# pkorus/neural-imaging

Hardware: AMD Instinct MI355X
Metric: patches/s (fwd+bwd) ISP->JPEG->FAN @256^2 (higher is better)
Workload: dtype bf16; 1 GPU; c4 = train_manipulation UNet->[native,sharpen:1,resample:50,gaussian:0.83,jpeg:80]->dJPEG(QF80,soft)->FAN, ds none, trainable nip+fan, lambda_nip 0.1; raw_patch=128, batch_per_gpu=64, global_batch=64, parallelism=dp1, world_size=1, hip_graph=False

## Files before the change

### include/nimg.h

```cpp
#ifndef NIMG_H
#define NIMG_H

#include <stddef.h>
#include <stdint.h>

#ifdef __cplusplus
extern "C" {
#endif

#define NIMG_OK 0
#define NIMG_ERR_ARG (-1)
#define NIMG_ERR_LAUNCH (-2)
#define NIMG_ERR_WORKSPACE (-3)

#define NIMG_BF16_IN 1
#define NIMG_BF16_OUT 2
#define NIMG_BF16_MASK 4
#define NIMG_BF16_DZ 8
#define NIMG_D2S_OUT 16
#define NIMG_MASK_CONV 128
#define NIMG_COPY_LRELU 64
#define NIMG_S2D_OUT 32
#define NIMG_UNPOOL_OUT 512
#define NIMG_D2S_CONVT 1024
// ... 252 lines not shown
                            float* out1, int o1, float* out2, int o2, const float* act_mask, int n, int h, int wd,
                            int ks, int stride, int pad_t, int pad_l, int pad_mode, int hout, int wout, int act,
                            float alpha, int flags, void* stream);
int nimg_conv2d_wgrad_bf16_ex(const float* in1, int c1, const float* in2, int c2, const float* dz, int cout, float* dw,
                              float* db, int n, int h, int wd, int ks, int stride, int pad_t, int pad_l, int pad_mode,
                              int hout, int wout, int accumulate, void* workspace, size_t workspace_bytes, int flags,
                              void* stream);
int nimg_conv2d_pool_fwd_bf16_ex(const float* in, int cin, const float* w, const void* wb, const float* bias,
                                 float* pool_out, unsigned char* pool_idx, int cout, int n, int h, int wd, int ks,
                                 int act, float alpha, int flags, void* stream);
int nimg_conv2d_fwd_pool_also_bf16(const float* in, int cin, const void* wb, const float* bias, float* out, float* pool_out,
                                   unsigned char* pool_idx, int cout, int n, int h, int wd, int act, float alpha, void* stream);
#define NIMG_ROWS_F32_OUT 1
int nimg_conv3_rows_bf16(const void* in1, int c1, const void* in2, int c2, const void* wb, const float* bias, const void* mask,
                         void* out, void* out2, void* pool_out, int n, int h, int wd, int cout, int act, float alpha, int flags,
                         void* stream);
int nimg_conv3_rows_d2s_bf16(const void* in, int c1, const void* wb, const float* bias, float* y, int n, int h, int wd, void* stream);
int nimg_conv3_rows_c4_bf16(const float* in, const float* w, const float* bias, void* out, int n, int h, int wd, int act, float alpha,
                            void* stream);

int nimg_conv2d_dgrad_unpool_out_bf16(const float* dz, int c1, const void* wb, const float* act, const float* skip, float* out,
                                      int cout, int n, int h, int wd, int apply_mask, float alpha, void* stream);
int nimg_conv2d_wgrad_pooled_bf16_ex(const float* in, int cin, const float* g, const unsigned char* idx, int cout,
                                     float* dw, float* db, int n, int h, int wd, int ks, int accumulate, void* workspace,
                                     size_t workspace_bytes, int flags, void* stream);
int nimg_conv2d_dgrad_fewin_pooled_bf16_ex(const float* g, const unsigned char* idx, const float* w, float* out, int ci,
                                           int cz, int n, int h, int wd, int ks, int flags, void* stream);
int nimg_maxpool2_unpool_ex(const float* dp, const unsigned char* idx, const float* pooled, float* dz, int n, int ho,
                            int wo, int c, int apply_lrelu_mask, float alpha, int flags, void* stream);
int nimg_convt2x2_fwd_bf16(const float* x, const void* wb, const float* bias, float* y, int n, int h, int wd, int cin,
                           int cout, void* stream);
int nimg_convt2x2_fwd_bf16_ex(const float* x, const void* wb, const float* bias, float* y, int n, int h, int wd, int cin,
                              int cout, int flags, void* stream);
int nimg_conv_weights_bf16_batch(const void* table, int n_entries, void* stream);
int nimg_conv2d_fwd_bf16(const float* in1, int c1, const float* in2, int c2, const void* wb, const float* bias,
                         float* out1, int o1, float* out2, int o2, const float* act_mask, int n, int h, int wd,
                         int ks, int stride, int pad_t, int pad_l, int pad_mode, int hout, int wout, int act,
                         float alpha, void* stream);
size_t nimg_conv2d_wgrad_bf16_workspace_bytes(int cin, int cout, int ks_h, int ks_w, int n, int hout, int wout);
int nimg_conv2d_wgrad_bf16(const float* in1, int c1, const float* in2, int c2, const float* dz, int cout, float* dw,
                           float* db, int n, int h, int wd, int ks, int stride, int pad_t, int pad_l, int pad_mode,
                           int hout, int wout, int accumulate, void* workspace, size_t workspace_bytes, void* stream);

int nimg_conv2d_fwd_smallc_bf16(const float* in, int cin, const float* w, const float* bias, float* out, int cout,
                                int n, int h, int wd, int ks, int pad_mode, int act, float alpha, void* stream);
int nimg_conv2d_fwd_smallc_bf16_ex(const float* in, int cin, const float* w, const float* bias, float* out, int cout,
                                   int n, int h, int wd, int ks, int pad_mode, int act, float alpha, int flags, void* stream);
int nimg_conv2d_dgrad_fewin_bf16(const float* dz, const float* w, float* out, int ci, int cz, int n, int h, int wd,
                                 int ks, void* stream);

int nimg_awgn_fwd(const float* x, const float* noise, float* y, uint8_t* mask, long count, float strength,
                  void* stream);
int nimg_awgn_bwd(const float* x, const float* noise, const float* dy, const uint8_t* mask, float* dx, long count,
                  float strength, void* stream);
int nimg_gamma_fwd(const float* x, float* y, long count, float gamma, void* stream);
int nimg_gamma_bwd(const float* x, const float* dy, float* dx, long count, float gamma, void* stream);
int nimg_median_fwd(const float* x, float* y, uint8_t* sel, int n, int h, int w, int kernel, void* stream);
int nimg_median_bwd(const float* dy, const uint8_t* sel, float* dx, int n, int h, int w, int kernel, void* stream);

#define NIMG_L3IC_E_READ 1
#define NIMG_L3IC_E_LANES 2
#define NIMG_L3IC_E_RANGE 4
#define NIMG_L3IC_E_SYMBOL 8
#define NIMG_L3IC_E_FREQ 16
#define NIMG_L3IC_E_VARINT 32
#define NIMG_L3IC_E_ODD 64
// ... 120 lines not shown
```

### neural-imaging_amd/csrc/common.h

```cpp
#pragma once
#include <hip/hip_runtime.h>
#include <stdint.h>
#include "../../include/nimg.h"

#define NIMG_CHECK_LAUNCH()                                   \
    do {                                                      \
        hipError_t e__ = hipGetLastError();                   \
        if (e__ != hipSuccess) return NIMG_ERR_LAUNCH;        \
    } while (0)

namespace nimg {

constexpr int WAVE = 64;

typedef __bf16 nimg_bf16x4 __attribute__((ext_vector_type(4)));

__device__ __forceinline__ float lrelu(float v, float alpha) { return v > 0.0f ? v : alpha * v; }

typedef unsigned short nimg_u16x2 __attribute__((ext_vector_type(2)));
__device__ __forceinline__ unsigned bf16x2_positive(unsigned packed) {
    const nimg_u16x2 one = {1, 1}, inf = {0x7F80, 0x7F80};
    const nimg_u16x2 u = __builtin_bit_cast(nimg_u16x2, packed) - one;
    return __builtin_bit_cast(unsigned, __builtin_elementwise_min(__builtin_elementwise_sub_sat(inf, u), one));
}
__device__ __forceinline__ unsigned sign_bits_interleave(unsigned x) {
    x = (x | (x << 4)) & 0x0F0F0F0Fu;
    x = (x | (x << 2)) & 0x33333333u;
    x = (x | (x << 1)) & 0x55555555u;
    return (x | (x >> 15)) & 0xFFFFu;
}

__device__ __forceinline__ float wave_sum(float v) {
#pragma unroll
    for (int o = 32; o > 0; o >>= 1) v += __shfl_xor(v, o, 64);
    return v;
}

__device__ __forceinline__ double wave_sum_d(double v) {
#pragma unroll
    for (int o = 32; o > 0; o >>= 1) v += __shfl_xor(v, o, 64);
    return v;
}

__device__ __forceinline__ bool map_coord(int& g, int size, int pad_mode) {
    const bool inside = (unsigned)g < (unsigned)size;
    const int sym = g < 0 ? -1 - g : 2 * size - 1 - g;
    const int ref = g < 0 ? -g : 2 * size - 2 - g;
    const int m = pad_mode == 1 ? sym : ref;
    const bool mapped = pad_mode != 0 && (unsigned)m < (unsigned)size;
    g = inside ? g : (mapped ? m : g);
    return inside || mapped;
}

__device__ __forceinline__ int xcd_order(int bid) {
#ifdef NIMG_NO_XCD_ORDER
    return bid;
#else
    const int g = (int)gridDim.x, x = bid & 7, r = g & 7;
    return x * (g >> 3) + (x < r ? x : r) + (bid >> 3);
#endif
}

typedef float nimg_f32x16 __attribute__((ext_vector_type(16)));

constexpr int EPI_PAD = 4;
template <int NI, bool BLOCK_SYNC = true, typename Emit>
__device__ __forceinline__ void epilogue_via_lds(const nimg_f32x16 (&acc)[NI], float* lds, int lane, Emit emit) {
    constexpr int RS = NI * 32 + EPI_PAD;
    const int half = lane >> 5, n = lane & 31;
    if (BLOCK_SYNC) __syncthreads();
    else __builtin_amdgcn_wave_barrier();
#pragma unroll
    for (int ni = 0; ni < NI; ++ni)
#pragma unroll
        for (int j = 0; j < 16; ++j) lds[((j & 3) + 8 * (j >> 2) + 4 * half) * RS + ni * 32 + n] = acc[ni][j];
    if (BLOCK_SYNC) __syncthreads();
    else __builtin_amdgcn_wave_barrier();
#pragma unroll
    for (int it = 0; it < (32 * NI * 8) / 64; ++it) {
        const int idx = it * 64 + lane, row = idx / (NI * 8), c4 = idx % (NI * 8);
        const float4 v = *reinterpret_cast<const float4*>(lds + row * RS + c4 * 4);
        emit(row, c4 * 4, v);
    }
}

template <int NI, bool BLOCK_SYNC = true, typename Bias, typename Emit>
__device__ __forceinline__ void pool_via_lds(const nimg_f32x16 (&acc)[NI], float* lds, int lane, float alpha, Bias bias4,
                                             Emit emit) {
    constexpr int RS = NI * 32 + EPI_PAD;
    const int half = lane >> 5, n = lane & 31;
    if (BLOCK_SYNC) __syncthreads();
    else __builtin_amdgcn_wave_barrier();
#pragma unroll
    for (int ni = 0; ni < NI; ++ni)
// ... 375 lines not shown
```

### neural-imaging_amd/csrc/conv_bf16_wgrad.hip

```cpp
#include "conv_bf16_wgrad.h"

namespace {

typedef short s16x4 __attribute__((ext_vector_type(4)));
typedef short s16x8 __attribute__((ext_vector_type(8)));

__device__ __forceinline__ bf16x8 tr_read8(const unsigned char* p0, const unsigned char* p1) {
    const s16x4 lo = __builtin_amdgcn_ds_read_tr16_b64_v4i16((s16x4 __attribute__((address_space(3)))*)p0);
    const s16x4 hi = __builtin_amdgcn_ds_read_tr16_b64_v4i16((s16x4 __attribute__((address_space(3)))*)p1);
    s16x8 r;
    r[0] = lo[0]; r[1] = lo[1]; r[2] = lo[2]; r[3] = lo[3]; r[4] = hi[0]; r[5] = hi[1]; r[6] = hi[2]; r[7] = hi[3];
    return *reinterpret_cast<bf16x8*>(&r);
}

constexpr int B_ZS = 192;

template <int KS, int STRIDE, int NW, bool INB, bool DZB, int TH, bool UNP = false, int NCO = 2, bool PAIR = false>
__global__ __launch_bounds__(NW * 64, 2) void conv_wgrad_bf16_kernel(const WgradParamsB p) {
    nimg::reduce_entry_inline(p.pre);
    constexpr int TCO = 32 * NCO, ZS = NCO == 2 ? B_ZS : 64, ZI = 4 * NCO;
    static_assert(NCO == 1 || NCO == 2, "one or two output fragments");
    static_assert(!UNP || NCO == 2, "un-pooling dz: 64-wide tile");
    static_assert(!UNP || (DZB && STRIDE == 1), "un-pooling dz: bf16-stored pooled gradient, stride 1");
    constexpr int TAPS = KS * KS, NT = (TAPS + NW - 1) / NW, NTHR = NW * 64;
    static_assert(!PAIR || (KS == 3 && STRIDE == 1 && TH == 8 && INB && DZB && !UNP), "image pairs: the 3x3 layers over 8 x 8 bf16 images");
    constexpr int THH = (TH - 1) * STRIDE + KS, TWH = PAIR ? 20 : (B_TW - 1) * STRIDE + KS;
    constexpr int NPIXH = THH * TWH, NPIX = TH * B_TW;
    static_assert(STRIDE == 1 || STRIDE == 2, "stride");
    extern __shared__ __attribute__((aligned(16))) unsigned char smem_raw[];
    unsigned char* sI = smem_raw;
    unsigned char* sZ = smem_raw + NPIXH * 64;
    const int tid = threadIdx.x, lane = tid & 63;
    const int wave = __builtin_amdgcn_readfirstlane(tid >> 6);
    const int Cin = p.C1 + p.C2;
    const int cib = (Cin + B_CI - 1) / B_CI, cob = (p.Cout + TCO - 1) / TCO;
    int bid = xcd_order(blockIdx.x);
    const int ci0 = (bid % cib) * B_CI;
    bid /= cib;
    const int co0 = (bid % cob) * TCO;
    const int split = bid / cob;
    const int half = lane >> 5, g = lane & 15, sub = (lane >> 4) & 1;

    f32x16 acc[NT][NCO];
#pragma unroll
    for (int t = 0; t < NT; ++t)
#pragma unroll
        for (int ni = 0; ni < NCO; ++ni)
#pragma unroll
            for (int j = 0; j < 16; ++j) acc[t][ni][j] = 0.0f;
    const int tiles = p.tiles_y * p.tiles_x;
    const int work_total = PAIR ? (p.N + 1) / 2 : p.N * tiles;
    const int w_begin = split * p.work_per_split;
    const int w_end = min(work_total, w_begin + p.work_per_split);
    const bool do_bias = p.db_partial && ci0 == 0;
    float bacc[8] = {0.f, 0.f, 0.f, 0.f, 0.f, 0.f, 0.f, 0.f};
    const int a_lane = ((half * (PAIR ? 10 : 8) + (g >> 2)) * STRIDE) * 64 + (sub * 16 + (g & 3) * 4) * 2;
    const int z_lane = (half * 8 + (g >> 2)) * ZS + (sub * 16 + (g & 3) * 4) * 2;
    constexpr int IP = (NPIXH * 4 + NTHR - 1) / NTHR, ZP = (NPIX * ZI) / NTHR;
    static_assert((NPIX * ZI) % NTHR == 0 && NTHR % ZI == 0, "dz tile must divide over the threads");
    float4 preI[IP][2], preZ[ZP][2];
    uint2 preZK[UNP ? ZP : 1];
    auto fetch = [&](int wk_) {
        const int n_ = (int)(wk_ / tiles), tile_ = (int)(wk_ % tiles);
        const int ty_ = (tile_ / p.tiles_x) * TH, tx_ = (tile_ % p.tiles_x) * B_TW;
        const int iy_ = ty_ * STRIDE - p.pad_t, ix_ = tx_ * STRIDE - p.pad_l;
#pragma unroll
        for (int q = 0; q < IP; ++q) {
            const int item = tid + q * NTHR;
            const int pix = item >> 2, c = ci0 + (item & 3) * 8;
            int gy = iy_ + pix / TWH, gx = ix_ + pix % TWH;
            int ni_ = n_;
            if constexpr (PAIR) {
                const int hx = pix % TWH;
                ni_ = 2 * wk_ + (hx >= 10 ? 1 : 0);
                gx = (hx >= 10 ? hx - 10 : hx) - 1;
                gy = pix / TWH - 1;
            }
            preI[q][0] = preI[q][1] = make_float4(0.f, 0.f, 0.f, 0.f);
            if (item < NPIXH * 4 && c < Cin && (!PAIR || ni_ < p.N) && map_coord(gy, p.H, p.pad_mode) && map_coord(gx, p.W, p.pad_mode)) {
                const long pixoff = ((long)ni_ * p.H + gy) * p.W + gx;
                if constexpr (INB) {
                    const __bf16* src = c < p.C1 ? reinterpret_cast<const __bf16*>(p.in1) + pixoff * p.C1 + c
                                                 : reinterpret_cast<const __bf16*>(p.in2) + pixoff * p.C2 + (c - p.C1);
                    preI[q][0] = *reinterpret_cast<const float4*>(src);
                } else {
                    const float* src = c < p.C1 ? p.in1 + pixoff * p.C1 + c : p.in2 + pixoff * p.C2 + (c - p.C1);
                    preI[q][0] = *reinterpret_cast<const float4*>(src);
// ... 111 lines not shown
        float* red = reinterpret_cast<float*>(smem_raw);
        if (wave > 0) {
#pragma unroll
            for (int ni = 0; ni < 2; ++ni)
#pragma unroll
                for (int j = 0; j < 16; ++j) red[(((wave - 1) * 2 + ni) * 16 + j) * 64 + lane] = acc[0][ni][j];
        }
        __syncthreads();
        if (wave == 0) {
#pragma unroll
            for (int w = 1; w < NW; ++w)
#pragma unroll
                for (int ni = 0; ni < 2; ++ni)
#pragma unroll
                    for (int j = 0; j < 16; ++j) acc[0][ni][j] += red[(((w - 1) * 2 + ni) * 16 + j) * 64 + lane];
        }
    }
    float* slab = p.partial + (long)split * TAPS * Cin * p.Cout;
#pragma unroll
    for (int t = 0; t < NT; ++t) {
        const int tap = KS == 1 ? 0 : wave + NW * t;
        if (tap >= TAPS || (KS == 1 && wave > 0)) continue;
#pragma unroll
        for (int ni = 0; ni < NCO; ++ni) {
            const int co = co0 + ni * 32 + (lane & 31);
            if (co >= p.Cout) continue;
#pragma unroll
            for (int j = 0; j < 16; ++j) {
                const int ci = ci0 + (j & 3) + 8 * (j >> 2) + 4 * half;
                if (ci < Cin) slab[((long)tap * Cin + ci) * p.Cout + co] = acc[t][ni][j];
            }
        }
    }
    if (p.tickets == nullptr) return;
    TicketJob job;
    job.cnt = p.tickets + (long)(xcd_order(blockIdx.x) % (cib * cob)) * ticket_words_per_tile_dev(p.splits, p.group);
    job.slab[0] = p.partial; job.stride[0] = (long)TAPS * Cin * p.Cout; job.dst[0] = p.dw;
    job.slab[1] = p.db_partial; job.stride[1] = p.Cout; job.dst[1] = p.db;
    job.splits = p.splits; job.group = p.group; job.accumulate = p.accumulate;
    const int rows = min(B_CI, Cin - ci0), c4n = min(TCO, p.Cout - co0) >> 2, Cout = p.Cout;
    const int witems = TAPS * rows * c4n;
    const int items = witems + ((p.db_partial && ci0 == 0) ? c4n : 0);
    ticket_finish<NTHR>(job, split, items, [=](int it) {
        TicketItem m;
        if (it >= witems) { m.which = 1; m.off = co0 + (it - witems) * 4; return m; }
        const int c4 = it % c4n, row = it / c4n;
        m.which = 0;
        m.off = ((long)(row / rows) * Cin + ci0 + row % rows) * Cout + co0 + c4 * 4;
        return m;
    }, reinterpret_cast<unsigned*>(smem_raw));
}

int splits_for(int cin, int cout, int n, int hout, int wout, int th = B_TH, int target_blocks = 512) {
    const long blocks_io = (long)cdiv(cin, B_CI) * cdiv(cout, B_CO);
    const long work = (long)n * cdiv(hout, th) * cdiv(wout, B_TW);
    long splits = (target_blocks + blocks_io - 1) / blocks_io;
    if (splits > work) splits = work;
    if (splits < 1) splits = 1;
    const long wps = (work + splits - 1) / splits;
    return (int)((work + wps - 1) / wps);
}

}

extern "C" {

size_t nimg_conv2d_wgrad_bf16_workspace_bytes(int cin, int cout, int ks_h, int ks_w, int n, int hout, int wout) {
    if (cin <= 0 || cout <= 0 || n <= 0) return 0;
    const size_t slab = (size_t)ks_h * ks_w * cin * cout * sizeof(float);
    const size_t generic = (slab + cout * sizeof(float)) * splits_for(cin, cout, n, hout, wout);
    const size_t packed = cin <= 4 ? (4 * slab + cout * sizeof(float)) * nimg_internal_wgrad_packed_splits(cout, n, hout, wout) : 0;
    const size_t tiny = (cin <= 4 && cout <= 4) ? nimg_internal_wgrad_tiny_bytes(ks_h, cin, cout) : 0;
    const size_t m = generic > packed ? generic : packed;
    return m > tiny ? m : tiny;
}

struct ReducePlan {
    nimg::ReduceEntry* defer = nullptr;
    const nimg::ReduceEntry* pre = nullptr;
};
static inline void finish_reduce2(const ReducePlan& plan, const float* p1, float* d1, long n1, int splits1, const float* p2,
                                  float* d2, long n2, int splits2, int accumulate, hipStream_t s) {
    if (plan.defer) nimg::fill_reduce_entry(plan.defer, p1, d1, n1, splits1, p2, d2, n2, splits2, accumulate);
    else launch_reduce2(p1, d1, n1, splits1, p2, d2, n2, splits2, accumulate, s);
}
struct OwedReduction {
    const nimg::ReduceEntry* e;
    hipStream_t s;
    void ran_in_kernel() { e = nullptr; }
    void now() {
        if (e && e->n1 > 0 && e->p1 && e->d1)
            launch_reduce2(e->p1, e->d1, e->n1, e->splits1, e->p2, e->d2, e->n2, e->splits2, e->accumulate, s);
        e = nullptr;
// ... 141 lines not shown
    } while (0)
    if (stride == 1 && ks == 1) NIMG_WGB(1, 1);
    else if (stride == 1 && ks == 3) NIMG_WGB(3, 1);
    else if (stride == 1 && ks == 5) NIMG_WGB(5, 1);
    else if (stride == 2 && ks == 2) NIMG_WGB(2, 2);
    else if (stride == 2 && ks == 5) NIMG_WGB(5, 2);
    else return NIMG_ERR_ARG;
#undef NIMG_WGB
#undef NIMG_WGB1
    NIMG_CHECK_LAUNCH();
    owed.ran_in_kernel();
    if (p.tickets) return NIMG_OK;
    finish_reduce2(plan, (const float*)workspace, dw, count, p.splits, db ? (const float*)p.db_partial : nullptr, db, (long)cout,
                   p.splits, accumulate, s);
    NIMG_CHECK_LAUNCH();
    return NIMG_OK;
}

int nimg_conv2d_wgrad_bf16(const float* in1, int c1, const float* in2, int c2, const float* dz, int cout, float* dw,
                           float* db, int n, int h, int wd, int ks, int stride, int pad_t, int pad_l, int pad_mode,
                           int hout, int wout, int accumulate, void* workspace, size_t workspace_bytes, void* stream) {
    return wgrad_bf16_impl(in1, c1, in2, c2, dz, nullptr, cout, dw, db, n, h, wd, ks, stride, pad_t, pad_l, pad_mode, hout,
                           wout, accumulate, workspace, workspace_bytes, 0, stream, ReducePlan{});
}

int nimg_conv2d_wgrad_bf16_ex(const float* in1, int c1, const float* in2, int c2, const float* dz, int cout, float* dw,
                              float* db, int n, int h, int wd, int ks, int stride, int pad_t, int pad_l, int pad_mode,
                              int hout, int wout, int accumulate, void* workspace, size_t workspace_bytes, int flags,
                              void* stream) {
    return wgrad_bf16_impl(in1, c1, in2, c2, dz, nullptr, cout, dw, db, n, h, wd, ks, stride, pad_t, pad_l, pad_mode, hout,
                           wout, accumulate, workspace, workspace_bytes, flags, stream, ReducePlan{});
}

int nimg_conv2d_wgrad_bf16_unpool(const void* in, int cin, const void* g, const unsigned char* idx, int cout, float* dw, float* db,
                                  int n, int h, int wd, int ks, int accumulate, void* workspace, size_t workspace_bytes,
                                  void* stream) {
    if (!idx || ks != 5 || (h & 1) || (wd & 1)) return NIMG_ERR_ARG;
    return wgrad_bf16_impl((const float*)in, cin, nullptr, 0, (const float*)g, idx, cout, dw, db, n, h, wd, ks, 1, 2, 2, 0, h, wd,
                           accumulate, workspace, workspace_bytes, NIMG_BF16_IN | NIMG_BF16_DZ, stream, ReducePlan{});
}

int nimg_conv2d_wgrad_bf16_deferred(const void* in1, int c1, const void* in2, int c2, const void* dz, const unsigned char* idx,
                                    int cout, float* dw, float* db, int n, int h, int wd, int ks, int stride, int pad_t, int pad_l,
                                    int pad_mode, int hout, int wout, void* workspace, size_t workspace_bytes, int flags,
                                    void* entry, void* stream) {
    if (!entry) return NIMG_ERR_ARG;
    nimg::ReduceEntry* e = reinterpret_cast<nimg::ReduceEntry*>(entry);
    nimg::fill_reduce_entry(e, nullptr, nullptr, 0, 0, nullptr, nullptr, 0, 0, 0);
    e->blocks1 = 0;
    return wgrad_bf16_impl((const float*)in1, c1, (const float*)in2, c2, (const float*)dz, idx, cout, dw, db, n, h, wd, ks, stride,
                           pad_t, pad_l, pad_mode, hout, wout, 0, workspace, workspace_bytes, flags, stream, ReducePlan{e, nullptr});
}

int nimg_conv2d_wgrad_bf16_chained(const void* in1, int c1, const void* in2, int c2, const void* dz, const unsigned char* idx,
                                   int cout, float* dw, float* db, int n, int h, int wd, int ks, int stride, int pad_t, int pad_l,
                                   int pad_mode, int hout, int wout, void* workspace, size_t workspace_bytes, int flags,
                                   const void* pre_entry, void* entry, void* stream) {
    if (!entry) return NIMG_ERR_ARG;
    nimg::ReduceEntry pre_copy;
    if (pre_entry) pre_copy = *reinterpret_cast<const nimg::ReduceEntry*>(pre_entry);
    nimg::ReduceEntry* e = reinterpret_cast<nimg::ReduceEntry*>(entry);
    *e = nimg::empty_reduce_entry();
    return wgrad_bf16_impl((const float*)in1, c1, (const float*)in2, c2, (const float*)dz, idx, cout, dw, db, n, h, wd, ks, stride,
                           pad_t, pad_l, pad_mode, hout, wout, 0, workspace, workspace_bytes, flags, stream,
                           ReducePlan{e, pre_entry ? &pre_copy : nullptr});
}
// ... 42 lines not shown
```

### neural-imaging_amd/csrc/conv_wgrad.hip

```cpp
#include "common.h"

namespace {

using namespace nimg;
typedef float f32x16 __attribute__((ext_vector_type(16)));

struct WgradParams {
    const float* in1;
    const float* in2;
    const float* dz;
    float* partial;
    float* db_partial;
    int C1, C2, Cout;
    int N, H, W, Hout, Wout, pad_t, pad_l;
    int tiles_y, tiles_x, splits, work_per_split, pad_mode;
    int tap0;
};

constexpr int WG_TH = 8, WG_TW = 16;
constexpr int CI_T = 32, CO_T = 64;

template <int KS, int STRIDE, bool VEC, int NW, int TCH = KS * KS>
__global__ __launch_bounds__(NW * 64, 2) void conv_wgrad_kernel(const WgradParams p) {
    constexpr int TAPS = KS * KS, NTHR = NW * 64;
    constexpr int NT = (TCH + NW - 1) / NW;
    constexpr bool PASSES = TCH < TAPS;
    const int tap_first = PASSES ? p.tap0 : 0, tap_end = PASSES ? min(TAPS, p.tap0 + TCH) : TAPS;
    constexpr int THH = (WG_TH - 1) * STRIDE + KS, TWH = (WG_TW - 1) * STRIDE + KS;
    constexpr int NPIXH = THH * TWH, NPIX = WG_TH * WG_TW;
    extern __shared__ __attribute__((aligned(16))) float smem[];
    float* sI = smem;
    float* sZ = smem + NPIXH * CI_T;

// ... 205 lines not shown
            if (co >= p.Cout) continue;
#pragma unroll
            for (int j = 0; j < 16; ++j) {
                const int i = (j & 3) + 8 * (j >> 2) + 4 * (lane >> 5);
                const int tl = i / CINP, ci = i % CINP, tap = f * TPF + tl;
                if (tl < TPF && tap < TAPS) slab[((long)tap * CINP + ci) * p.Cout + co] = acc[f][ni][j];
            }
        }
}

__global__ __launch_bounds__(256) void bias_grad_partial_kernel(const float* __restrict__ dz,
                                                                float* __restrict__ partial, long npix, int cout,
                                                                long pix_per_block) {
    extern __shared__ float red[];
    const int tid = threadIdx.x;
    const int cpad = cout >= 256 ? 256 : (cout > 128 ? 256 : (cout > 64 ? 128 : (cout > 32 ? 64 : 32)));
    const int phases = 256 / cpad;
    const int c = tid % cpad, ph = tid / cpad;
    const long p0 = (long)blockIdx.x * pix_per_block, p1 = min(npix, p0 + pix_per_block);
    for (int cb = 0; cb < cout; cb += cpad) {
        float s = 0.f;
        if (cb + c < cout)
            for (long px = p0 + ph; px < p1; px += phases) s += dz[px * cout + cb + c];
        red[tid] = s;
        __syncthreads();
        if (ph == 0 && cb + c < cout) {
            for (int k = 1; k < phases; ++k) s += red[k * cpad + c];
            partial[(long)blockIdx.x * cout + cb + c] = s;
        }
        __syncthreads();
    }
}

typedef __bf16 bg_bf16x4 __attribute__((ext_vector_type(4)));
template <bool BF>
struct BiasSrc {
    const void* base;
    __device__ __forceinline__ float4 operator[](long i) const {
        if constexpr (BF) {
            const bg_bf16x4 v = reinterpret_cast<const bg_bf16x4*>(base)[i];
            return make_float4((float)v[0], (float)v[1], (float)v[2], (float)v[3]);
        } else {
            return reinterpret_cast<const float4*>(base)[i];
        }
    }
};
template <bool BF>
__global__ __launch_bounds__(256) void bias_grad_partial4_kernel(const float* __restrict__ dz,
                                                                 float* __restrict__ partial, long npix, int cout,
                                                                 long pix_per_block) {
    __shared__ float4 red4[256];
    const int tid = threadIdx.x, cq = cout >> 2, phases = 256 / cq;
    const int c = tid % cq, ph = tid / cq;
    const long p0 = (long)blockIdx.x * pix_per_block, p1 = min(npix, p0 + pix_per_block);
    const BiasSrc<BF> srcb{dz};
    float4 a0 = make_float4(0.f, 0.f, 0.f, 0.f), a1 = a0, a2 = a0, a3 = a0;
    long px = p0 + ph;
    for (; px + 3L * phases < p1; px += 4L * phases) {
        const float4 v0 = srcb[px * cq + c], v1 = srcb[(px + phases) * cq + c], v2 = srcb[(px + 2L * phases) * cq + c],
                     v3 = srcb[(px + 3L * phases) * cq + c];
        a0.x += v0.x; a0.y += v0.y; a0.z += v0.z; a0.w += v0.w;
        a1.x += v1.x; a1.y += v1.y; a1.z += v1.z; a1.w += v1.w;
        a2.x += v2.x; a2.y += v2.y; a2.z += v2.z; a2.w += v2.w;
        a3.x += v3.x; a3.y += v3.y; a3.z += v3.z; a3.w += v3.w;
    }
    for (; px < p1; px += phases) {
        const float4 v = srcb[px * cq + c];
        a0.x += v.x; a0.y += v.y; a0.z += v.z; a0.w += v.w;
    }
    red4[tid] = make_float4((a0.x + a1.x) + (a2.x + a3.x), (a0.y + a1.y) + (a2.y + a3.y),
                            (a0.z + a1.z) + (a2.z + a3.z), (a0.w + a1.w) + (a2.w + a3.w));
    __syncthreads();
    if (ph == 0) {
        float4 s = red4[c];
        for (int k = 1; k < phases; ++k) {
            const float4 v = red4[k * cq + c];
            s.x += v.x; s.y += v.y; s.z += v.z; s.w += v.w;
        }
        reinterpret_cast<float4*>(partial + (long)blockIdx.x * cout)[c] = s;
    }
}

}

extern "C" {

static int wgrad_splits(int cin, int cout, int n, int hout, int wout) {
    const long blocks_io = (long)nimg::cdiv(cin, CI_T) * nimg::cdiv(cout, CO_T);
    const long work = (long)n * nimg::cdiv(hout, WG_TH) * nimg::cdiv(wout, WG_TW);
    long splits = (512 + blocks_io - 1) / blocks_io;
    if (splits > work) splits = work;
    if (splits < 1) splits = 1;
    const long wps = (work + splits - 1) / splits;
    return (int)((work + wps - 1) / wps);
}

static int packed_splits(int cout, int n, int hout, int wout) {
    const long blocks_io = nimg::cdiv(cout, cout <= 32 ? 32 : 64);
    const long work = (long)n * nimg::cdiv(hout, WG_TH) * nimg::cdiv(wout, WG_TW);
    long splits = (512 + blocks_io - 1) / blocks_io;
    if (splits > work) splits = work;
    if (splits < 1) splits = 1;
    const long wps = (work + splits - 1) / splits;
    return (int)((work + wps - 1) / wps);
}

size_t nimg_conv2d_wgrad_workspace_bytes(int cin, int cout, int ks_h, int ks_w, int n, int hout, int wout) {
    if (cin <= 0 || cout <= 0 || n <= 0) return 0;
    const size_t slab = (size_t)ks_h * ks_w * cin * cout * sizeof(float);
    const size_t generic = (slab + cout * sizeof(float)) * wgrad_splits(cin, cout, n, hout, wout);
    const size_t packed = cin <= 4 ? (4 * slab + cout * sizeof(float)) * packed_splits(cout, n, hout, wout) : 0;
    const size_t tiny = (cin <= 4 && cout <= 4) ? nimg_internal_wgrad_tiny_bytes(ks_h, cin, cout) : 0;
    const size_t m = generic > packed ? generic : packed;
// ... 75 lines not shown
                auto k = conv_wgrad_kernel<KS_, 1, true, 8, TCH_>;                                            \
                (void)hipFuncSetAttribute((const void*)k, hipFuncAttributeMaxDynamicSharedMemorySize, (int)lds);  \
                hipLaunchKernelGGL(k, dim3((unsigned)blocks), dim3(512), lds, s, p);                          \
            } else {                                                                                          \
                auto k = conv_wgrad_kernel<KS_, 1, false, 8, TCH_>;                                           \
                (void)hipFuncSetAttribute((const void*)k, hipFuncAttributeMaxDynamicSharedMemorySize, (int)lds);  \
                hipLaunchKernelGGL(k, dim3((unsigned)blocks), dim3(512), lds, s, p);                          \
            }                                                                                                 \
        }                                                                                                     \
    } while (0)
    p.tap0 = 0;
    if (stride == 1 && ks == 1) NIMG_WG(1, 1);
    else if (stride == 1 && ks == 3) NIMG_WG(3, 1);
    else if (stride == 1 && ks == 5) NIMG_WG(5, 1);
    else if (stride == 2 && ks == 2) NIMG_WG(2, 2);
    else if (stride == 2 && ks == 5) NIMG_WG(5, 2);
    else if (stride == 1 && ks == 4) NIMG_WG(4, 1);
    else if (stride == 1 && ks == 6) NIMG_WG_BIG(6);
    else if (stride == 1 && ks == 8) NIMG_WG_BIG(8);
    else if (stride == 1 && ks == 10) NIMG_WG_BIG(10);
    else if (stride == 1 && ks == 7) NIMG_WG_BIG(7);
    else if (stride == 1 && ks == 9) NIMG_WG_BIG(9);
    else if (stride == 1 && ks == 11) NIMG_WG_BIG(11);
    else return NIMG_ERR_ARG;
#undef NIMG_WG
#undef NIMG_WG_BIG
    NIMG_CHECK_LAUNCH();
    nimg::launch_reduce2((const float*)workspace, dw, count, p.splits, db ? (const float*)p.db_partial : nullptr, db,
                         (long)cout, p.splits, accumulate, s);
    NIMG_CHECK_LAUNCH();
    return NIMG_OK;
}

static long bias_grad_blocks(long npix) { return npix < 512 ? 1 : (npix / 512 > 2048 ? 2048 : npix / 512); }

size_t nimg_bias_grad_workspace_bytes(long npix, int cout) {
    return (size_t)bias_grad_blocks(npix) * cout * sizeof(float);
}

int nimg_bias_grad(const float* dz, float* db, long npix, int cout, int accumulate, void* workspace,
                   size_t workspace_bytes, void* stream) {
    return nimg_bias_grad_ex(dz, db, npix, cout, accumulate, workspace, workspace_bytes, 0, stream);
}

int nimg_bias_grad_ex(const float* dz, float* db, long npix, int cout, int accumulate, void* workspace,
                      size_t workspace_bytes, int flags, void* stream) {
    if (!dz || !db || npix <= 0 || cout <= 0 || !workspace || (flags & ~NIMG_BF16_DZ)) return NIMG_ERR_ARG;
    if ((flags & NIMG_BF16_DZ) && !((cout & 3) == 0 && (cout >> 2) <= 256 && 256 % (cout >> 2) == 0)) return NIMG_ERR_ARG;
    if (workspace_bytes < nimg_bias_grad_workspace_bytes(npix, cout)) return NIMG_ERR_WORKSPACE;
    const long blocks = bias_grad_blocks(npix);
    const long ppb = (npix + blocks - 1) / blocks;
    hipStream_t s = (hipStream_t)stream;
    if (flags & NIMG_BF16_DZ)
        hipLaunchKernelGGL(bias_grad_partial4_kernel<true>, dim3((unsigned)blocks), dim3(256), 0, s, dz, (float*)workspace,
                           npix, cout, ppb);
    else if ((cout & 3) == 0 && (cout >> 2) <= 256 && 256 % (cout >> 2) == 0)
        hipLaunchKernelGGL(bias_grad_partial4_kernel<false>, dim3((unsigned)blocks), dim3(256), 0, s, dz, (float*)workspace,
                           npix, cout, ppb);
    else
        hipLaunchKernelGGL(bias_grad_partial_kernel, dim3((unsigned)blocks), dim3(256), 256 * sizeof(float), s, dz,
                           (float*)workspace, npix, cout, ppb);
    NIMG_CHECK_LAUNCH();
    nimg::launch_reduce2((const float*)workspace, db, (long)cout, (int)blocks, nullptr, nullptr, 0, 0, accumulate, s);
    NIMG_CHECK_LAUNCH();
    return NIMG_OK;
}

}
```

### neural-imaging_amd/models/layers.py

```python
import numpy as np
import torch

from .. import ops
from ..helpers import kernels as hk


FUSED_ACTIVATIONS = (None, 'leaky_relu')


def act_forward(y, activation):
    if isinstance(y, tuple):
        raise RuntimeError('a bf16 copy cannot be combined with activation {}'.format(activation))
    return ops.activation(y, activation, out=y)


class Conv2D(object):

    def __init__(self, name, ks, cin, cout, activation=None, stride=1, cin2=0, mask_activation='leaky_relu'):
        self.name, self.ks, self.cin, self.cin2, self.cout = name, ks, cin, cin2, cout
        self.activation, self.stride = activation, stride
        self.mask_activation = mask_activation

    def specs(self):
        return [(self.name + '/kernel', (self.ks, self.ks, self.cin + self.cin2, self.cout)),
# ... 92 lines not shown
                       out_bf16=s2d_out)
        return (y if fused else act_forward(y, self.activation)), xs

    def backward_params_image(self, store, ctx, dz):
        if ctx.dtype != torch.bfloat16:
            return self.backward_params(store, ctx, dz)
        with ops.side_stream(ctx, dz, key=store.g[self.name + '/kernel'].data_ptr()):
            dw3 = ops.conv2d_wgrad(ctx, dz, 3, db=store.g[self.name + '/bias'])
            ops.s2d_conv_weights_bwd(dw3, store.g[self.name + '/kernel'])

    def backward_input_image(self, store, dz, in_hw, a):
        return ops.conv2d_dgrad_strided2(dz, store.p[self.name + '/kernel'], in_hw, scale=a)


class Conv2DTranspose2x2(object):

    def __init__(self, name, cin, cout):
        self.name, self.cin, self.cout = name, cin, cout

    def specs(self):
        return [(self.name + '/kernel', (2, 2, self.cout, self.cin)), (self.name + '/bias', (self.cout,))]

    def init(self, store, gen):
        from .tfmodel import glorot_uniform_
        k = torch.empty((2, 2, self.cout, self.cin), dtype=torch.float32)
        glorot_uniform_(k, self.cin * 4, self.cout * 4, gen)
        store.p[self.name + '/kernel'].copy_(k)
        store.p[self.name + '/bias'].zero_()

    def forward(self, store, x, out_bf16=False):
        return ops.convt2x2(x, store.p[self.name + '/kernel'], store.p[self.name + '/bias'], out_bf16=out_bf16)

    def backward_params(self, store, x, dy):
        ops.convt2x2_wgrad(x, dy, dw=store.g[self.name + '/kernel'], side=True)
        ops.bias_grad(dy, db=store.g[self.name + '/bias'], side=True)

    def backward_input(self, store, dy, act_mask=None, out_bf16=False, mask_activation='leaky_relu'):
        if act_mask is not None and mask_activation not in FUSED_ACTIVATIONS:
            d = ops.convt2x2_dgrad(dy, store.p[self.name + '/kernel'])
            return ops.activation_bwd(d, act_mask, mask_activation, out=d)
        return ops.convt2x2_dgrad(dy, store.p[self.name + '/kernel'], act_mask=act_mask, out_bf16=out_bf16)


class ConstrainedConv2D(object):

    def __init__(self, name='constrained', filter_strength=100.0):
        self.name, self.strength = name, float(filter_strength)

    def specs(self):
        return [(self.name + '/kernel', (5, 5, 3, 3))]

    def init(self, store, gen=None):
        store.p[self.name + '/kernel'].copy_(torch.from_numpy(hk.residual_init_filter().astype(np.float32)))
        if hasattr(store, 'register_constrained'):
            store.register_constrained(self.name + '/kernel', self.strength)

    _flip = (None, None)

    def forward(self, store, x, c4_only=False):
        cc = getattr(store, 'constrained', None)
        if ops.ADAM_IMAGES and ops.ADAM_CCONV and ops.COMPUTE == 'bf16' and cc is not None and \
                cc['kernel'] is store.p[self.name + '/kernel'] and cc['strength'] == self.strength:
            nf, flip = store.constrained_filter()
            self._flip = (nf, flip)
        else:
            nf = ops.constrained_kernel(store.p[self.name + '/kernel'], self.strength)
            self._flip = (None, None)
        y, c4 = ops.cconv3(x, nf, pad_mode=1, want_f32=not c4_only, want_c4=c4_only)
# ... 14 lines not shown
```

### neural-imaging_amd/ops.py

```python
import math
import os

import numpy as np
import torch

from . import _lib

LRELU_ALPHA = 0.2

COMPUTE = 'f32'


STORE_BF16 = True


COMPUTE_EPOCH = 0


def set_compute(mode):
    global COMPUTE, COMPUTE_EPOCH
    if mode not in ('f32', 'bf16'):
        raise ValueError('compute mode must be f32 or bf16')
    if mode != COMPUTE:
        COMPUTE_EPOCH += 1
# ... 824 lines not shown
    need = _lib.load().nimg_bias_grad_workspace_bytes(npix, cout)
    ws = _ws_current(dz.device).get(need, dz.device)
    _lib.call('nimg_bias_grad_ex', _p(dz), _p(db), npix, cout, 1 if accumulate else 0, _p(ws), ws.numel(),
              BF16_DZ if _is_bf16(dz) else 0, _stream())
    return db


def convt2x2(x, w, bias, out_bf16=False):
    _f32(w, bias)
    _fb(x)
    n, h, wd, cin = x.shape
    cout = w.shape[2]
    y = torch.empty((n, 2 * h, 2 * wd, cout), dtype=torch.bfloat16 if out_bf16 else torch.float32, device=x.device)
    if COMPUTE == 'bf16' and cin % 8 == 0 and cout >= 8:
        wb = weights_bf16(w, 1)
        _lib.call('nimg_convt2x2_fwd_bf16_ex', _p(x), _p(wb), _p(bias), _p(y), n, h, wd, cin, cout,
                  (BF16_IN if _is_bf16(x) else 0) | (BF16_OUT if out_bf16 else 0), _stream())
        return y
    if _is_bf16(x) or out_bf16:
        raise RuntimeError('bf16-stored tensor reached a float32 transposed-convolution path')
    _lib.call('nimg_convt2x2_fwd', _p(x), _p(w), _p(bias), _p(y), n, h, wd, cin, cout, _stream())
    return y


def convt2x2_dgrad(dy, w, act_mask=None, out_bf16=False):
    n, h2, w2, _ = dy.shape
    return conv2d(dy, w, None, stride=2, pads=(0, 0), out_hw=(h2 // 2, w2 // 2), act_mask=act_mask, out_bf16=out_bf16)


def convt2x2_wgrad(x, dy, dw=None, side=False):
    return conv2d_wgrad(dy, x, 2, stride=2, pads=(0, 0), dw=dw, side=side)


def maxpool2(x):
    _fb(x)
    n, h, w, c = x.shape
    y = torch.empty((n, h // 2, w // 2, c), dtype=x.dtype, device=x.device)
    if _is_bf16(x):
        _lib.call('nimg_maxpool2_fwd_bf16', _p(x), _p(y), n, h, w, c, _stream())
        return y
    _lib.call('nimg_maxpool2_fwd', _p(x), _p(y), n, h, w, c, _stream())
    return y


def maxpool2_bwd(dp, yact, add=None, apply_mask=True, out=None, alpha=None):
    a = LRELU_ALPHA if alpha is None else float(alpha)
    _fb(dp, yact, add, out)
    n, h, w, c = yact.shape
    dz = torch.empty_like(yact) if out is None else out
    if _is_bf16(yact):
        if any(t is not None and not _is_bf16(t) for t in (dp, add, dz)):
            raise RuntimeError('maxpool2_bwd on a bf16-stored activation needs bf16-stored gradients')
        _lib.call('nimg_maxpool2_bwd_bf16', _p(dp), _p(yact), _p(add), _p(dz), n, h, w, c, 1 if apply_mask else 0,
                  a, _stream())
        return dz
    _f32(dp, add, dz)
    _lib.call('nimg_maxpool2_bwd', _p(dp), _p(yact), _p(add), _p(dz), n, h, w, c, 1 if apply_mask else 0,
              a, _stream())
    return dz


ACT_SIGN = os.environ.get('NIMG_NO_ACT_SIGN') is None


def conv2d_pool_sign_ok(x, w, out_bf16=True):
    n, h, wd, cin = x.shape
# ... 1686 lines not shown
```

Before: 8173 patches/s.

## Fuse transposed-conv weight and bias gradients into one wgrad launch with bias riders

Adds a combined convt2x2 parameter-gradient entry point that runs the bf16 wgrad GEMM kernel with extra 'rider' blocks computing bias partial sums in the same grid, followed by a single shared reduction for dw and db. This replaces separate wgrad and bias_grad launches, each with its own reduction, to cut launch overhead and let the bias reduction overlap the GEMM blocks. The bias-partial code is factored into a shared header. The fused path is skipped when tickets or a reduce carrier are active, in which case it falls back to the old calls.

```diff
diff --git a/include/nimg.h b/include/nimg.h
--- a/include/nimg.h
+++ b/include/nimg.h
@@ -308,6 +308,9 @@
                            int cout, void* stream);
 int nimg_convt2x2_fwd_bf16_ex(const float* x, const void* wb, const float* bias, float* y, int n, int h, int wd, int cin,
                               int cout, int flags, void* stream);
+size_t nimg_convt2x2_params_bf16_workspace_bytes(int n, int h, int wd, int cin, int cout);
+int nimg_convt2x2_params_bf16(const void* x, const void* dy, float* dw, float* db, int n, int h, int wd, int cin, int cout,
+                              int accumulate, void* workspace, size_t workspace_bytes, void* stream);
 int nimg_conv_weights_bf16_batch(const void* table, int n_entries, void* stream);
 int nimg_conv2d_fwd_bf16(const float* in1, int c1, const float* in2, int c2, const void* wb, const float* bias,
                          float* out1, int o1, float* out2, int o2, const float* act_mask, int n, int h, int wd,
diff --git a/neural-imaging_amd/csrc/bias_grad.h b/neural-imaging_amd/csrc/bias_grad.h
--- /dev/null
+++ b/neural-imaging_amd/csrc/bias_grad.h
@@ -0,0 +1,57 @@
+#pragma once
+#include "common.h"
+
+namespace nimg {
+
+static inline long bias_grad_blocks(long npix) { return npix < 512 ? 1 : (npix / 512 > 2048 ? 2048 : npix / 512); }
+static inline bool bias_partial4_ok(int cout) { return (cout & 3) == 0 && (cout >> 2) <= 256 && 256 % (cout >> 2) == 0; }
+
+typedef __bf16 bg_bf16x4 __attribute__((ext_vector_type(4)));
+template <bool BF>
+struct BiasSrc {
+    const void* base;
+    __device__ __forceinline__ float4 operator[](long i) const {
+        if constexpr (BF) {
+            const bg_bf16x4 v = reinterpret_cast<const bg_bf16x4*>(base)[i];
+            return make_float4((float)v[0], (float)v[1], (float)v[2], (float)v[3]);
+        } else {
+            return reinterpret_cast<const float4*>(base)[i];
+        }
+    }
+};
+
+template <bool BF>
+__device__ __forceinline__ void bias_partial4_block(const void* __restrict__ dz, float* __restrict__ partial, long npix, int cout,
+                                                    long pix_per_block, long block, float4* red4) {
+    const int tid = threadIdx.x, cq = cout >> 2, phases = 256 / cq;
+    const int c = tid % cq, ph = tid / cq;
+    const long p0 = block * pix_per_block, p1 = min(npix, p0 + pix_per_block);
+    const BiasSrc<BF> srcb{dz};
+    float4 a0 = make_float4(0.f, 0.f, 0.f, 0.f), a1 = a0, a2 = a0, a3 = a0;
+    long px = p0 + ph;
+    for (; px + 3L * phases < p1; px += 4L * phases) {
+        const float4 v0 = srcb[px * cq + c], v1 = srcb[(px + phases) * cq + c], v2 = srcb[(px + 2L * phases) * cq + c],
+                     v3 = srcb[(px + 3L * phases) * cq + c];
+        a0.x += v0.x; a0.y += v0.y; a0.z += v0.z; a0.w += v0.w;
+        a1.x += v1.x; a1.y += v1.y; a1.z += v1.z; a1.w += v1.w;
+        a2.x += v2.x; a2.y += v2.y; a2.z += v2.z; a2.w += v2.w;
+        a3.x += v3.x; a3.y += v3.y; a3.z += v3.z; a3.w += v3.w;
+    }
+    for (; px < p1; px += phases) {
+        const float4 v = srcb[px * cq + c];
+        a0.x += v.x; a0.y += v.y; a0.z += v.z; a0.w += v.w;
+    }
+    red4[tid] = make_float4((a0.x + a1.x) + (a2.x + a3.x), (a0.y + a1.y) + (a2.y + a3.y),
+                            (a0.z + a1.z) + (a2.z + a3.z), (a0.w + a1.w) + (a2.w + a3.w));
+    __syncthreads();
+    if (ph == 0) {
+        float4 s = red4[c];
+        for (int k = 1; k < phases; ++k) {
+            const float4 v = red4[k * cq + c];
+            s.x += v.x; s.y += v.y; s.z += v.z; s.w += v.w;
+        }
+        reinterpret_cast<float4*>(partial + block * cout)[c] = s;
+    }
+}
+
+}
diff --git a/neural-imaging_amd/csrc/common.h b/neural-imaging_amd/csrc/common.h
--- a/neural-imaging_amd/csrc/common.h
+++ b/neural-imaging_amd/csrc/common.h
@@ -52,14 +52,15 @@
     return inside || mapped;
 }
 
-__device__ __forceinline__ int xcd_order(int bid) {
+__device__ __forceinline__ int xcd_order_of(int bid, int g) {
 #ifdef NIMG_NO_XCD_ORDER
     return bid;
 #else
-    const int g = (int)gridDim.x, x = bid & 7, r = g & 7;
+    const int x = bid & 7, r = g & 7;
     return x * (g >> 3) + (x < r ? x : r) + (bid >> 3);
 #endif
 }
+__device__ __forceinline__ int xcd_order(int bid) { return xcd_order_of(bid, (int)gridDim.x); }
 
 typedef float nimg_f32x16 __attribute__((ext_vector_type(16)));
 
diff --git a/neural-imaging_amd/csrc/conv_bf16_wgrad.hip b/neural-imaging_amd/csrc/conv_bf16_wgrad.hip
--- a/neural-imaging_amd/csrc/conv_bf16_wgrad.hip
+++ b/neural-imaging_amd/csrc/conv_bf16_wgrad.hip
@@ -1,4 +1,5 @@
 #include "conv_bf16_wgrad.h"
+#include "bias_grad.h"
 
 namespace {
 
@@ -14,10 +15,11 @@
 }
 
 constexpr int B_ZS = 192;
-
-template <int KS, int STRIDE, int NW, bool INB, bool DZB, int TH, bool UNP = false, int NCO = 2, bool PAIR = false>
+constexpr int CONVT_MAX_RIDERS = 256;
+
+template <int KS, int STRIDE, int NW, bool INB, bool DZB, int TH, bool UNP = false, int NCO = 2, bool PAIR = false, bool RIDER = false>
 __global__ __launch_bounds__(NW * 64, 2) void conv_wgrad_bf16_kernel(const WgradParamsB p) {
-    nimg::reduce_entry_inline(p.pre);
+    if constexpr (!RIDER) nimg::reduce_entry_inline(p.pre);
     constexpr int TCO = 32 * NCO, ZS = NCO == 2 ? B_ZS : 64, ZI = 4 * NCO;
     static_assert(NCO == 1 || NCO == 2, "one or two output fragments");
     static_assert(!UNP || NCO == 2, "un-pooling dz: 64-wide tile");
@@ -27,6 +29,7 @@
     constexpr int THH = (TH - 1) * STRIDE + KS, TWH = PAIR ? 20 : (B_TW - 1) * STRIDE + KS;
     constexpr int NPIXH = THH * TWH, NPIX = TH * B_TW;
     static_assert(STRIDE == 1 || STRIDE == 2, "stride");
+    static_assert(!RIDER || (INB && !UNP && !PAIR), "bias riders: a bf16-stored input, plain tiles");
     extern __shared__ __attribute__((aligned(16))) unsigned char smem_raw[];
     unsigned char* sI = smem_raw;
     unsigned char* sZ = smem_raw + NPIXH * 64;
@@ -34,7 +37,19 @@
     const int wave = __builtin_amdgcn_readfirstlane(tid >> 6);
     const int Cin = p.C1 + p.C2;
     const int cib = (Cin + B_CI - 1) / B_CI, cob = (p.Cout + TCO - 1) / TCO;
-    int bid = xcd_order(blockIdx.x);
+    int bid;
+    if constexpr (RIDER) {
+        const int wgb = cib * cob * p.splits, riders = (int)gridDim.x - wgb;
+        if ((int)blockIdx.x >= wgb) {
+            const long npix = (long)p.N * p.H * p.W;
+            nimg::bias_partial4_block<true>(p.in1, p.db_partial, npix, p.C1, (npix + riders - 1) / riders, (long)blockIdx.x - wgb,
+                                            reinterpret_cast<float4*>(smem_raw));
+            return;
+        }
+        bid = xcd_order_of(blockIdx.x, wgb);
+    } else {
+        bid = xcd_order(blockIdx.x);
+    }
     const int ci0 = (bid % cib) * B_CI;
     bid /= cib;
     const int co0 = (bid % cob) * TCO;
@@ -52,7 +67,7 @@
     const int work_total = PAIR ? (p.N + 1) / 2 : p.N * tiles;
     const int w_begin = split * p.work_per_split;
     const int w_end = min(work_total, w_begin + p.work_per_split);
-    const bool do_bias = p.db_partial && ci0 == 0;
+    const bool do_bias = !RIDER && p.db_partial && ci0 == 0;
     float bacc[8] = {0.f, 0.f, 0.f, 0.f, 0.f, 0.f, 0.f, 0.f};
     const int a_lane = ((half * (PAIR ? 10 : 8) + (g >> 2)) * STRIDE) * 64 + (sub * 16 + (g & 3) * 4) * 2;
     const int z_lane = (half * 8 + (g >> 2)) * ZS + (sub * 16 + (g & 3) * 4) * 2;
@@ -230,7 +245,7 @@
             }
         }
     }
-    if (p.tickets == nullptr) return;
+    if (RIDER || p.tickets == nullptr) return;
     TicketJob job;
     job.cnt = p.tickets + (long)(xcd_order(blockIdx.x) % (cib * cob)) * ticket_words_per_tile_dev(p.splits, p.group);
     job.slab[0] = p.partial; job.stride[0] = (long)TAPS * Cin * p.Cout; job.dst[0] = p.dw;
@@ -257,6 +272,12 @@
     if (splits < 1) splits = 1;
     const long wps = (work + splits - 1) / splits;
     return (int)((work + wps - 1) / wps);
+}
+
+__global__ __launch_bounds__(256) void convt_bias_partial4_kernel(const void* __restrict__ dy, float* __restrict__ partial, long npix,
+                                                                  int cout, long pix_per_block) {
+    __shared__ float4 red4[256];
+    nimg::bias_partial4_block<true>(dy, partial, npix, cout, pix_per_block, (long)blockIdx.x, red4);
 }
 
 }
@@ -464,6 +485,61 @@
                            wout, accumulate, workspace, workspace_bytes, flags, stream, ReducePlan{});
 }
 
+static bool convt_params_shape_ok(int n, int h, int wd, int cin, int cout) {
+    return n > 0 && h > 0 && wd > 0 && cin > 0 && cout >= 8 && (cin & 7) == 0 && (cout & 7) == 0 && nimg::bias_partial4_ok(cout) &&
+           (long)n * cdiv(h, B_TH) * cdiv(wd, B_TW) < (1L << 31);
+}
+
+size_t nimg_convt2x2_params_bf16_workspace_bytes(int n, int h, int wd, int cin, int cout) {
+    if (!convt_params_shape_ok(n, h, wd, cin, cout)) return 0;
+    const size_t slab = (size_t)4 * cin * cout * sizeof(float);
+    return nimg::align256(slab * splits_for(cout, cin, n, h, wd)) +
+           (size_t)nimg::bias_grad_blocks((long)n * 4 * h * wd) * cout * sizeof(float);
+}
+
+int nimg_convt2x2_params_bf16(const void* x, const void* dy, float* dw, float* db, int n, int h, int wd, int cin, int cout,
+                              int accumulate, void* workspace, size_t workspace_bytes, void* stream) {
+    if (!x || !dy || !dw || !db || !workspace || !convt_params_shape_ok(n, h, wd, cin, cout)) return NIMG_ERR_ARG;
+    if (workspace_bytes < nimg_convt2x2_params_bf16_workspace_bytes(n, h, wd, cin, cout)) return NIMG_ERR_WORKSPACE;
+    WgradParamsB p;
+    p.pre = nimg::empty_reduce_entry();
+    p.in1 = (const float*)dy; p.in2 = nullptr; p.dz = (const float*)x; p.dz_idx = nullptr; p.partial = (float*)workspace;
+    p.flags = NIMG_BF16_IN | NIMG_BF16_DZ;
+    p.tickets = nullptr; p.dw = nullptr; p.db = nullptr; p.group = 1; p.accumulate = accumulate;
+    p.C1 = cout; p.C2 = 0; p.Cout = cin; p.N = n; p.H = 2 * h; p.W = 2 * wd; p.Hout = h; p.Wout = wd;
+    p.pad_t = 0; p.pad_l = 0; p.pad_mode = 0;
+    p.tiles_y = cdiv(h, B_TH); p.tiles_x = cdiv(wd, B_TW);
+    p.splits = splits_for(cout, cin, n, h, wd);
+    const long work = (long)n * p.tiles_y * p.tiles_x;
+    p.work_per_split = (int)((work + p.splits - 1) / p.splits);
+    const long count = (long)4 * cin * cout;
+    const long npix = (long)n * p.H * p.W;
+    const long riders = nimg::bias_grad_blocks(npix);
+    float* dbp = (float*)((char*)workspace + nimg::align256((size_t)p.splits * count * sizeof(float)));
+    const long blocks = (long)cdiv(cout, B_CI) * cdiv(cin, B_CO) * p.splits;
+    constexpr size_t lds = (size_t)(2 * B_TH) * (2 * B_TW) * 64 + (size_t)B_TH * B_TW * B_ZS;
+    hipStream_t s = (hipStream_t)stream;
+    if (riders <= CONVT_MAX_RIDERS) {
+        p.db_partial = dbp;
+        auto k = conv_wgrad_bf16_kernel<2, 2, 4, true, true, B_TH, false, 2, false, true>;
+        (void)hipFuncSetAttribute((const void*)k, hipFuncAttributeMaxDynamicSharedMemorySize, (int)lds);
+        hipLaunchKernelGGL(k, dim3((unsigned)(blocks + riders)), dim3(256), lds, s, p);
+        NIMG_CHECK_LAUNCH();
+    } else {
+        p.db_partial = nullptr;
+        auto k = conv_wgrad_bf16_kernel<2, 2, 4, true, true, B_TH>;
+        (void)hipFuncSetAttribute((const void*)k, hipFuncAttributeMaxDynamicSharedMemorySize, (int)lds);
+        hipLaunchKernelGGL(k, dim3((unsigned)blocks), dim3(256), lds, s, p);
+        NIMG_CHECK_LAUNCH();
+        hipLaunchKernelGGL(convt_bias_partial4_kernel, dim3((unsigned)riders), dim3(256), 0, s, dy, dbp, npix, cout,
+                           (npix + riders - 1) / riders);
+        NIMG_CHECK_LAUNCH();
+    }
+    launch_reduce2((const float*)workspace, dw, count, p.splits, dbp, db, (long)cout, (int)riders, accumulate, s);
+    NIMG_CHECK_LAUNCH();
+    return NIMG_OK;
+}
+
 int nimg_conv2d_wgrad_bf16_unpool(const void* in, int cin, const void* g, const unsigned char* idx, int cout, float* dw, float* db,
                                   int n, int h, int wd, int ks, int accumulate, void* workspace, size_t workspace_bytes,
                                   void* stream) {
diff --git a/neural-imaging_amd/csrc/conv_wgrad.hip b/neural-imaging_amd/csrc/conv_wgrad.hip
--- a/neural-imaging_amd/csrc/conv_wgrad.hip
+++ b/neural-imaging_amd/csrc/conv_wgrad.hip
@@ -1,4 +1,5 @@
 #include "common.h"
+#include "bias_grad.h"
 
 namespace {
 
@@ -270,53 +271,12 @@
     }
 }
 
-typedef __bf16 bg_bf16x4 __attribute__((ext_vector_type(4)));
-template <bool BF>
-struct BiasSrc {
-    const void* base;
-    __device__ __forceinline__ float4 operator[](long i) const {
-        if constexpr (BF) {
-            const bg_bf16x4 v = reinterpret_cast<const bg_bf16x4*>(base)[i];
-            return make_float4((float)v[0], (float)v[1], (float)v[2], (float)v[3]);
-        } else {
-            return reinterpret_cast<const float4*>(base)[i];
-        }
-    }
-};
 template <bool BF>
 __global__ __launch_bounds__(256) void bias_grad_partial4_kernel(const float* __restrict__ dz,
                                                                  float* __restrict__ partial, long npix, int cout,
                                                                  long pix_per_block) {
     __shared__ float4 red4[256];
-    const int tid = threadIdx.x, cq = cout >> 2, phases = 256 / cq;
-    const int c = tid % cq, ph = tid / cq;
-    const long p0 = (long)blockIdx.x * pix_per_block, p1 = min(npix, p0 + pix_per_block);
-    const BiasSrc<BF> srcb{dz};
-    float4 a0 = make_float4(0.f, 0.f, 0.f, 0.f), a1 = a0, a2 = a0, a3 = a0;
-    long px = p0 + ph;
-    for (; px + 3L * phases < p1; px += 4L * phases) {
-        const float4 v0 = srcb[px * cq + c], v1 = srcb[(px + phases) * cq + c], v2 = srcb[(px + 2L * phases) * cq + c],
-                     v3 = srcb[(px + 3L * phases) * cq + c];
-        a0.x += v0.x; a0.y += v0.y; a0.z += v0.z; a0.w += v0.w;
-        a1.x += v1.x; a1.y += v1.y; a1.z += v1.z; a1.w += v1.w;
-        a2.x += v2.x; a2.y += v2.y; a2.z += v2.z; a2.w += v2.w;
-        a3.x += v3.x; a3.y += v3.y; a3.z += v3.z; a3.w += v3.w;
-    }
-    for (; px < p1; px += phases) {
-        const float4 v = srcb[px * cq + c];
-        a0.x += v.x; a0.y += v.y; a0.z += v.z; a0.w += v.w;
-    }
-    red4[tid] = make_float4((a0.x + a1.x) + (a2.x + a3.x), (a0.y + a1.y) + (a2.y + a3.y),
-                            (a0.z + a1.z) + (a2.z + a3.z), (a0.w + a1.w) + (a2.w + a3.w));
-    __syncthreads();
-    if (ph == 0) {
-        float4 s = red4[c];
-        for (int k = 1; k < phases; ++k) {
-            const float4 v = red4[k * cq + c];
-            s.x += v.x; s.y += v.y; s.z += v.z; s.w += v.w;
-        }
-        reinterpret_cast<float4*>(partial + (long)blockIdx.x * cout)[c] = s;
-    }
+    bias_partial4_block<BF>(dz, partial, npix, cout, pix_per_block, (long)blockIdx.x, red4);
 }
 
 }
@@ -458,10 +418,8 @@
     return NIMG_OK;
 }
 
-static long bias_grad_blocks(long npix) { return npix < 512 ? 1 : (npix / 512 > 2048 ? 2048 : npix / 512); }
-
 size_t nimg_bias_grad_workspace_bytes(long npix, int cout) {
-    return (size_t)bias_grad_blocks(npix) * cout * sizeof(float);
+    return (size_t)nimg::bias_grad_blocks(npix) * cout * sizeof(float);
 }
 
 int nimg_bias_grad(const float* dz, float* db, long npix, int cout, int accumulate, void* workspace,
@@ -472,15 +430,15 @@
 int nimg_bias_grad_ex(const float* dz, float* db, long npix, int cout, int accumulate, void* workspace,
                       size_t workspace_bytes, int flags, void* stream) {
     if (!dz || !db || npix <= 0 || cout <= 0 || !workspace || (flags & ~NIMG_BF16_DZ)) return NIMG_ERR_ARG;
-    if ((flags & NIMG_BF16_DZ) && !((cout & 3) == 0 && (cout >> 2) <= 256 && 256 % (cout >> 2) == 0)) return NIMG_ERR_ARG;
+    if ((flags & NIMG_BF16_DZ) && !nimg::bias_partial4_ok(cout)) return NIMG_ERR_ARG;
     if (workspace_bytes < nimg_bias_grad_workspace_bytes(npix, cout)) return NIMG_ERR_WORKSPACE;
-    const long blocks = bias_grad_blocks(npix);
+    const long blocks = nimg::bias_grad_blocks(npix);
     const long ppb = (npix + blocks - 1) / blocks;
     hipStream_t s = (hipStream_t)stream;
     if (flags & NIMG_BF16_DZ)
         hipLaunchKernelGGL(bias_grad_partial4_kernel<true>, dim3((unsigned)blocks), dim3(256), 0, s, dz, (float*)workspace,
                            npix, cout, ppb);
-    else if ((cout & 3) == 0 && (cout >> 2) <= 256 && 256 % (cout >> 2) == 0)
+    else if (nimg::bias_partial4_ok(cout))
         hipLaunchKernelGGL(bias_grad_partial4_kernel<false>, dim3((unsigned)blocks), dim3(256), 0, s, dz, (float*)workspace,
                            npix, cout, ppb);
     else
diff --git a/neural-imaging_amd/models/layers.py b/neural-imaging_amd/models/layers.py
--- a/neural-imaging_amd/models/layers.py
+++ b/neural-imaging_amd/models/layers.py
@@ -148,8 +148,7 @@
         return ops.convt2x2(x, store.p[self.name + '/kernel'], store.p[self.name + '/bias'], out_bf16=out_bf16)
 
     def backward_params(self, store, x, dy):
-        ops.convt2x2_wgrad(x, dy, dw=store.g[self.name + '/kernel'], side=True)
-        ops.bias_grad(dy, db=store.g[self.name + '/bias'], side=True)
+        ops.convt2x2_params(x, dy, store.g[self.name + '/kernel'], store.g[self.name + '/bias'], side=True)
 
     def backward_input(self, store, dy, act_mask=None, out_bf16=False, mask_activation='leaky_relu'):
         if act_mask is not None and mask_activation not in FUSED_ACTIVATIONS:
diff --git a/neural-imaging_amd/ops.py b/neural-imaging_amd/ops.py
--- a/neural-imaging_amd/ops.py
+++ b/neural-imaging_amd/ops.py
@@ -880,6 +880,33 @@
     return conv2d_wgrad(dy, x, 2, stride=2, pads=(0, 0), dw=dw, side=side)
 
 
+CONVT_GEMM = os.environ.get('NIMG_NO_CONVT_GEMM') is None
+
+
+def convt2x2_params(x, dy, dw, db, side=False, accumulate=False):
+    _f32(dw, db)
+    _fb(x, dy)
+    n, h, wd, cin = x.shape
+    cout = dy.shape[3]
+    carried = TICKETS or (side and _SIDE['enabled'] and _reduce_carrier() is not None)
+    need = 0
+    if CONVT_GEMM and COMPUTE == 'bf16' and _is_bf16(x) and _is_bf16(dy) and not carried:
+        need = _lib.load().nimg_convt2x2_params_bf16_workspace_bytes(n, h, wd, cin, cout)
+    if not need:
+        conv2d_wgrad(dy, x, 2, stride=2, pads=(0, 0), dw=dw, accumulate=accumulate, side=side)
+        bias_grad(dy, db=db, accumulate=accumulate, side=side)
+        return dw, db
+    if side and _SIDE['enabled']:
+        _side_index(dw.data_ptr())
+        _side_index(db.data_ptr())
+        with _on_side_stream(x, dy, key=dw.data_ptr()):
+            return convt2x2_params(x, dy, dw, db, side=False, accumulate=accumulate)
+    ws = _ws_current(x.device).get(need, x.device)
+    _lib.call('nimg_convt2x2_params_bf16', _p(x), _p(dy), _p(dw), _p(db), n, h, wd, cin, cout, 1 if accumulate else 0, _p(ws),
+              ws.numel(), _stream())
+    return dw, db
+
+
 def maxpool2(x):
     _fb(x)
     n, h, w, c = x.shape
```

Result: slower. 7926 patches/s (-3.0%).
